# jd-opensource/xllm

Hardware: AMD Instinct MI355X
Metric: decode tokens/s, Qwen2-7B int8 bs=256 ctx=4096 (higher is better)
Workload: dtype int8; 1 GPU; qwen2_7b W8A8 int8 decode step, global_batch=256 ctx=4096, paged KV block=128 bf16, 28 layers + lm_head + argmax, random-init weights; global_batch=256, ctx=4096, per_gpu_batch=256, block_table=random placement of every sequence's pages in a pool of 1.1 x the pages in use, parallelism=tp1, layout=single, quant_fusion=True, micro_batches=1, hip_graph=True

## Files before the change

### xllm_amd/_lib.py

```python
from __future__ import annotations

import ctypes as C
import os

_HERE = os.path.dirname(os.path.abspath(__file__))
LIB_PATH = os.environ.get("XLLM_MI355_LIB") or os.path.join(_HERE, "lib", "libxllm_mi355.so")

vp, i64, i32, f32, sz = C.c_void_p, C.c_int64, C.c_int32, C.c_float, C.c_size_t
ci = C.c_int
u64 = C.c_uint64



class DecodeMetadata(C.Structure):
    _fields_ = ([(n, vp) for n in (
        "src_tokens", "src_positions", "src_new_cache_slots", "src_kv_seq_lens", "src_paged_kv_indptr",
        "src_paged_kv_indices", "src_paged_kv_last_page_len", "dst_tokens", "dst_positions", "dst_new_cache_slots",
        "dst_kv_seq_lens", "dst_kv_seq_lens_delta", "dst_paged_kv_indptr", "dst_paged_kv_indices",
        "dst_paged_kv_last_page_len")] +
        [(n, i64) for n in ("actual_num_tokens", "padded_num_tokens", "actual_batch_size", "actual_indices_size")] +
        [("dst_block_table", vp), ("dst_kv_lens", vp), ("max_blocks_per_seq", i64), ("padded_batch_size", i64)])



# ... 47 lines not shown
    "xllm_mi355_act_and_mul_dynamic_int8_quant": ([vp, vp, vp, i64, i64, ci, ci, vp], ci),
    "xllm_mi355_act_and_mul_dynamic_int8_quant_live": ([vp, vp, vp, i64, i64, ci, ci, vp, i64, vp], ci),
    "xllm_mi355_scaled_quantize": ([vp, vp, vp, i64, i64, ci, vp], ci),
    "xllm_mi355_scaled_matmul": ([vp, vp, vp, vp, vp, vp, vp, i64, i64, i64, ci, vp], ci),
    "xllm_mi355_scaled_matmul_add": ([vp, vp, vp, vp, vp, vp, vp, i64, i64, i64, ci, vp], ci),
    "xllm_mi355_add16": ([vp, vp, vp, i64, ci, vp], ci),
    "xllm_mi355_set_gemm_workspace": ([vp, sz], ci),
    "xllm_mi355_set_gemm_workspace_for_stream": ([vp, vp, sz], ci),
    "xllm_mi355_scaled_matmul_add_rms_norm": ([vp, vp, vp, vp, vp, vp, vp, f32, vp, vp, vp, i64, i64, i64, ci, vp], ci),
    "xllm_mi355_pack_weight_i8": ([vp, vp, i64, i64, vp], ci),
    "xllm_mi355_scaled_matmul_packed": ([vp, vp, vp, vp, vp, vp, vp, i64, i64, i64, ci, vp, sz, vp], ci),
    "xllm_mi355_scaled_matmul_add_rms_norm_packed": ([vp, vp, vp, vp, vp, vp, vp, f32, vp, vp, vp, i64, i64, i64, ci, vp, sz,
                                                      vp], ci),
    "xllm_mi355_scaled_matmul_gate_up_act": ([vp, vp, vp, vp, vp, vp, vp, vp, i64, i64, i64, ci, vp, sz, vp], ci),
    "xllm_mi355_quantize_with_row_amax": ([vp, vp, vp, vp, i64, i64, ci, vp], ci),
    "xllm_mi355_static_scaled_fp8_quant": ([vp, vp, vp, i64, ci, vp], ci),
    "xllm_mi355_fp8_scaled_quantize": ([vp, vp, vp, vp, i64, ci, vp], ci),
    "xllm_mi355_fp8_scaled_quantize_ws": ([vp, vp, vp, i64, ci, vp, sz, vp], ci),
    "xllm_mi355_fp8_scaled_matmul": ([vp, vp, vp, i64, vp, i64, vp, vp, i64, i64, i64, ci, vp], ci),
    "xllm_mi355_pack_weight_fp8": ([vp, vp, i64, i64, vp], ci),
    "xllm_mi355_fp8_scaled_matmul_packed": ([vp, vp, vp, i64, vp, i64, vp, vp, i64, i64, i64, ci, vp, sz, vp], ci),
    "xllm_mi355_matmul": ([vp, vp, vp, vp, i64, i64, i64, ci, vp], ci),
    "xllm_mi355_pack_weight_16": ([vp, vp, i64, i64, vp], ci),
    "xllm_mi355_matmul_packed": ([vp, vp, vp, vp, i64, i64, i64, ci, vp, sz, vp], ci),
    "xllm_mi355_matmul_gate_up_act": ([vp, vp, vp, vp, i64, i64, i64, ci, vp, sz, vp], ci),
    "xllm_mi355_matmul_argmax_workspace_bytes": ([i64, i64], sz),
    "xllm_mi355_matmul_argmax_packed": ([vp, vp, vp, vp, vp, i64, i64, i64, ci, vp, sz, vp], ci),
    "xllm_mi355_prefill_attention": ([vp, vp, vp, vp, vp, vp, i64, i64, i64, i64, i64, i64, i64, i64, f32, ci, i64,
                                      ci, vp], ci),
    "xllm_mi355_paged_decode_attention_int8": ([vp, vp, vp, vp, vp, vp, vp, vp, i64, i64, i64, i64, i64, i64, i64, i64,
# ... 76 lines not shown
```

### xllm_amd/csrc/gemm.hip

```cpp
#include <stdlib.h>

#include "gemm_types.h"

namespace xm {

constexpr int BM = 128, BN = 128, BKB = 128;

template <int KIND, bool SPLITK, int KB, int MINW>
__global__ __launch_bounds__(256, MINW) void gemm_kernel(const uint8_t* __restrict__ A_, const uint8_t* __restrict__ W_,
                                                      int M_, int N, int64_t Kb, int m_tiles, int n_tiles,
                                                      int ksteps_per_split, GemmEpi epi) {
  const uint8_t* A = A_;
  const uint8_t* W = W_;
  int M = M_;
  void* out_base = epi.out;
  using MT = MmaTraits<KIND>;
  using acc_t = typename MT::acc_t;
  constexpr int CPR = KB / 16;
  constexpr int NST = BM * CPR / 256;
  __shared__ __attribute__((aligned(16))) uint8_t lds[2][2][BM * KB];
  auto SW = [](int row) { return CPR == 8 ? ((row >> 1) & 7) : ((row >> 2) & 3); };

  const int tid = threadIdx.x, lane = tid & 63, wave = tid >> 6;
  const int wm = wave >> 1, wn = wave & 1;
// ... 771 lines not shown
  if (N % 256 != 0 || K % 128 != 0 || ((uintptr_t)a % 16) || ((uintptr_t)act_out % 16) || ((uintptr_t)w_scale % 16))
    return XM_ERR_UNSUPPORTED;
  if (M == 0) return XM_OK;
  GemmEpi epi{a_scale, M, w_scale, N, bias, nullptr, nullptr, dtype == XM_BF16, nullptr, 0};
  epi.gate_up = 1;
  epi.act_out = act_out;
  epi.row_amax = row_amax;
  if (w_packed && M <= 512) {
    const int rc = launch_gemm_ws_i8(a, w_packed, M, N, K, epi, workspace, ws_bytes, nullptr, (hipStream_t)stream);
    if (rc != XM_ERR_UNSUPPORTED) return rc;
  }
  if (!w || ((uintptr_t)w % 16)) return XM_ERR_UNSUPPORTED;
  return launch_gemm_p8<kI8>(a, w, M, N, K, epi, nullptr, 0, 1, (hipStream_t)stream);
}

int xllm_mi355_fp8_scaled_matmul(const uint8_t* a, const uint8_t* w, const float* a_scale, int64_t a_scale_numel,
                                 const float* w_scale, int64_t w_scale_numel, const void* bias, void* out, int64_t M,
                                 int64_t N, int64_t K, int out_dtype, void* stream) {
  if (!a || !w || !a_scale || !w_scale || !out || M < 0 || N < 0 || K <= 0) return XM_ERR_INVALID;
  if (out_dtype != XM_BF16 && out_dtype != XM_F16) return XM_ERR_UNSUPPORTED;
  if ((a_scale_numel != 1 && a_scale_numel != M) || (w_scale_numel != 1 && w_scale_numel != N)) return XM_ERR_INVALID;
  if (K % 128 != 0 || ((uintptr_t)a % 16) || ((uintptr_t)w % 16)) return XM_ERR_UNSUPPORTED;
  GemmEpi epi{a_scale, a_scale_numel, w_scale, w_scale_numel, bias, out, nullptr, out_dtype == XM_BF16, nullptr, 0};
  void* ws = nullptr;
  size_t ws_bytes = 0;
  gemm_ws_for(stream, &ws, &ws_bytes);
  return launch_gemm<kFP8>(a, w, M, N, K, epi, ws, ws_bytes, (hipStream_t)stream);
}

int xllm_mi355_pack_weight_fp8(const uint8_t* w, uint8_t* packed, int64_t N, int64_t K, void* stream) {
// ... 172 lines not shown
```

### xllm_amd/csrc/gemm_types.h

```cpp
#pragma once
#include <type_traits>

#include "common.h"

namespace xm {

typedef int i32x4_t __attribute__((ext_vector_type(4)));
typedef int i32x16_t __attribute__((ext_vector_type(16)));
typedef float f32x16_t __attribute__((ext_vector_type(16)));
typedef __bf16 gbf16x8_t __attribute__((ext_vector_type(8)));
typedef _Float16 gf16x8_t __attribute__((ext_vector_type(8)));

enum GemmKind { kI8 = 0, kFP8 = 1, kBF16 = 2, kF16 = 3 };

template <int KIND>
struct MmaTraits;
template <>
struct MmaTraits<kI8> {
  using acc_t = i32x16_t;
  static __device__ __forceinline__ acc_t zero() { return acc_t{0}; }
  static __device__ __forceinline__ acc_t mma(const uint4& a, const uint4& b, acc_t c) {
    i32x4_t av = {(int)a.x, (int)a.y, (int)a.z, (int)a.w}, bv = {(int)b.x, (int)b.y, (int)b.z, (int)b.w};
    return __builtin_amdgcn_mfma_i32_32x32x32_i8(av, bv, c, 0, 0, 0);
  }
// ... 47 lines not shown
  const int32_t* group_tiles;
  const int32_t* gather_rows;
  int gather_div;
  int gather_src_rows;
  int gate_up;
  void* act_out;
  float* row_amax;
  int w_policy;
  float* argmax_val;
  int32_t* argmax_idx;
  int argmax_slots;
  int slab_nt;
  int out_nt;
  const void* addend;
  int group_inline;
};

__device__ __forceinline__ bool argmax_better(float v, int i, float bv, int bi) {
  const bool vn = v != v, bn = bv != bv;
  if (vn || bn) return vn && (!bn || i < bi);
  return v > bv || (v == bv && i < bi);
}

struct GroupSlot { int e, off, cnt, tile; };
__device__ __forceinline__ bool group_locate(const GemmEpi& epi, int m_slots, int n_tiles, int bm, int lane, int& mt, int& nt,
                                             GroupSlot& gs) {
  const int b = blockIdx.x, xcd = b & 7, j = b >> 3;
  int used;
  int ct = 0, cr = 0, it = 0, ir = 0;
  int c4[4] = {0, 0, 0, 0};
// ... 149 lines not shown
               : "+v"(F[0]), "+v"(F[1]), "+v"(F[2]), "+v"(F[3]), "+v"(F[4]), "+v"(F[5]), "+v"(F[6]), "+v"(F[7]))

template <int KIND>
int launch_gemm_p8(const void* A, const void* W, int64_t M, int64_t N, int64_t Kb, GemmEpi epi, void* workspace,
                   size_t ws_bytes, int splits, hipStream_t s);

int launch_gemm_ws_i8(const void* A, const void* Wp, int64_t M, int64_t N, int64_t K, GemmEpi epi, void* workspace,
                      size_t ws_bytes, int* n_slabs, hipStream_t s);
int launch_gemm_ws_fp8(const void* A, const void* Wp, int64_t M, int64_t N, int64_t K, GemmEpi epi, void* workspace,
                       size_t ws_bytes, hipStream_t s);
int launch_gemm_ws_h16(const void* A, const void* Wp, int64_t M, int64_t N, int64_t Kb, GemmEpi epi, void* workspace,
                       size_t ws_bytes, hipStream_t s);
int launch_gemm_ws_h16_argmax(const void* A, const void* Wp, int64_t M, int64_t N, int64_t Kb, GemmEpi epi, int64_t* out_idx,
                              float* out_val, void* workspace, size_t ws_bytes, hipStream_t s);
int launch_pack_weight_i8(const void* W, void* Wp, int64_t N, int64_t K, hipStream_t s);

template <typename T>
int launch_gemm_wsb_dense(const void* x, const void* w, const void* bias, void* out, int64_t M, int64_t N, int64_t K,
                          void* workspace, size_t ws_bytes, hipStream_t s);
template <typename T>
int launch_gemm_wsb_grouped(const void* x, const void* w, const int32_t* counts, void* out, int64_t max_rows,
                            int64_t n_experts, int64_t N, int64_t K, const int32_t* row_index, int64_t index_div,
                            hipStream_t s);

}
```

### xllm_amd/csrc/gemm_ws.hip

```cpp
#include <stdlib.h>

#include "gemm_types.h"

namespace xm {

constexpr int WS_BK = 128;
constexpr int WS_FRAG = 1024;
#ifndef WS_W_AUX
#define WS_W_AUX 2
#endif

__global__ __launch_bounds__(256) void pack_weight_i8_kernel(const uint8_t* __restrict__ W, uint8_t* __restrict__ Wp,
                                                             int64_t N, int64_t K) {
  const int64_t chunks_per_row = K / 16, total = N * chunks_per_row;
  const int64_t KT = K / WS_BK;
  for (int64_t i = (int64_t)blockIdx.x * blockDim.x + threadIdx.x; i < total; i += (int64_t)gridDim.x * blockDim.x) {
    const int64_t n = i / chunks_per_row, c = i - n * chunks_per_row;
    const int64_t g = n >> 4, r = n & 15, kt = c >> 3, ks = (c >> 2) & 1, kq = c & 3;
    const uint4 v = *reinterpret_cast<const uint4*>(W + n * K + c * 16);
    *reinterpret_cast<uint4*>(Wp + ((g * KT + kt) * 2 + ks) * WS_FRAG + (kq * 16 + r) * 16) = v;
  }
}

#define WS_BUFLOAD(DST, VOFF, RSRC, SOFF, IMM)                                             \
// ... 15 lines not shown
  int so_a, so_w;
  ws_lds_ptr_t dump;
  int nvalid_w;
  int w_nt;
};
template <int NDA, int NDW, int WNT = -1>
__device__ __forceinline__ void ws_dma_piece(const WsDma& d, const int (&voff_a)[8], const int (&voff_w)[8], int j) {
  if (j < NDA) __builtin_amdgcn_raw_ptr_buffer_load_lds(d.rsrc_a, d.dst_a + j * WS_FRAG, 16, voff_a[j], d.so_a, 0, 0);
  else if (WNT == 1 || (WNT < 0 && d.w_nt))
    __builtin_amdgcn_raw_ptr_buffer_load_lds(d.rsrc_w, (j - NDA) < d.nvalid_w ? d.dst_w + (j - NDA) * WS_FRAG : d.dump, 16,
                                             voff_w[j - NDA], d.so_w, 0, WS_W_AUX);
  else
    __builtin_amdgcn_raw_ptr_buffer_load_lds(d.rsrc_w, (j - NDA) < d.nvalid_w ? d.dst_w + (j - NDA) * WS_FRAG : d.dump, 16,
                                             voff_w[j - NDA], d.so_w, 0, 0);
}
template <int NDA, int NDW, int NG>
__device__ __forceinline__ void ws_dma_slot(const WsDma& d, const int (&voff_a)[8], const int (&voff_w)[8], int slot) {
  constexpr int ND = NDA + NDW;
  const int lo = slot * ND / (2 * NG), hi = (slot + 1) * ND / (2 * NG);
#pragma unroll
  for (int j = lo; j < hi; ++j) ws_dma_piece<NDA, NDW>(d, voff_a, voff_w, j);
}

template <int NDA, int NDW, int LO, int HI, int WNT = -1>
__device__ __forceinline__ void ws_dma_range(const WsDma& d, const int (&voff_a)[8], const int (&voff_w)[8], int slot, int nslots) {
  const int lo = LO + slot * (HI - LO) / nslots, hi = LO + (slot + 1) * (HI - LO) / nslots;
#pragma unroll
  for (int j = lo; j < hi; ++j) ws_dma_piece<NDA, NDW, WNT>(d, voff_a, voff_w, j);
}

template <int MB, int NG, int NDA, int NDW, int NG_LEFT>
__device__ __forceinline__ void ws_kstep1(i32x4_t (&acc)[MB][NG], u32x4 (&fw)[NG], const u32x4 (&a1)[MB], const WsDma& d,
                                          const int (&voff_a)[8], const int (&voff_w)[8]) {
  if constexpr (NG_LEFT > 0) {
    constexpr int ng = NG - NG_LEFT;
    asm volatile("s_waitcnt lgkmcnt(%1)" : "+v"(fw[ng]) : "n"(NG_LEFT - 1));
#pragma unroll
    for (int mb = 0; mb < MB; ++mb) WS_MFMA(acc[mb][ng], fw[ng], a1[mb]);
    ws_dma_slot<NDA, NDW, NG>(d, voff_a, voff_w, NG + ng);
    ws_kstep1<MB, NG, NDA, NDW, NG_LEFT - 1>(acc, fw, a1, d, voff_a, voff_w);
  }
}
template <int MB, int NG, int NDA, int NDW>
__device__ __forceinline__ void ws_compute(i32x4_t (&acc)[MB][NG], unsigned rw, unsigned ra0, unsigned ra1, const WsDma& d,
                                           const int (&voff_a)[8], const int (&voff_w)[8]) {
  u32x4 a0[MB], a1[MB], fw[NG];
#pragma unroll
  for (int mb = 0; mb < MB; ++mb) WS_DSR(a0[mb], ra0, mb * 16 * WS_BK);
#pragma unroll
  for (int mb = 0; mb < MB; ++mb) WS_DSR(a1[mb], ra1, mb * 16 * WS_BK);
#pragma unroll
  for (int ng = 0; ng < NG; ++ng) WS_DSR(fw[ng], rw, ng * 2 * WS_FRAG);
#pragma unroll
  for (int ng = 0; ng < NG; ++ng) {
    if (ng == 0) {
      if constexpr (MB == 4)
        asm volatile("s_waitcnt lgkmcnt(%5)" : "+v"(a0[0]), "+v"(a0[1]), "+v"(a0[2]), "+v"(a0[3]), "+v"(fw[0]) : "n"(NG - 1));
      else
        asm volatile("s_waitcnt lgkmcnt(%3)" : "+v"(a0[0]), "+v"(a0[1]), "+v"(fw[0]) : "n"(NG - 1));
    } else {
      asm volatile("s_waitcnt lgkmcnt(%1)" : "+v"(fw[ng]) : "n"(NG - 1));
    }
#pragma unroll
    for (int mb = 0; mb < MB; ++mb) WS_MFMA(acc[mb][ng], fw[ng], a0[mb]);
    WS_DSR(fw[ng], rw, ng * 2 * WS_FRAG + WS_FRAG);
    ws_dma_slot<NDA, NDW, NG>(d, voff_a, voff_w, ng);
  }
  if constexpr (MB == 4) asm volatile("" : "+v"(a1[0]), "+v"(a1[1]), "+v"(a1[2]), "+v"(a1[3]));
  else asm volatile("" : "+v"(a1[0]), "+v"(a1[1]));
  ws_kstep1<MB, NG, NDA, NDW, NG>(acc, fw, a1, d, voff_a, voff_w);
  __builtin_amdgcn_sched_barrier(0);
}


typedef float f32x4_t __attribute__((ext_vector_type(4)));
__device__ __forceinline__ f32x4_t ws_mma_fp8(const u32x4 w0, const u32x4 w1, const u32x4 a0, const u32x4 a1, f32x4_t c) {
  const gi32x8_t wv = {(int)w0.x, (int)w0.y, (int)w0.z, (int)w0.w, (int)w1.x, (int)w1.y, (int)w1.z, (int)w1.w};
  const gi32x8_t av = {(int)a0.x, (int)a0.y, (int)a0.z, (int)a0.w, (int)a1.x, (int)a1.y, (int)a1.z, (int)a1.w};
  return __builtin_amdgcn_mfma_scale_f32_16x16x128_f8f6f4(wv, av, c, 0, 0, 0, 0, 0, 0);
}
template <int NDA, int NDW, int NSLOTS>
__device__ __forceinline__ void ws_dma_slot_n(const WsDma& d, const int (&voff_a)[8], const int (&voff_w)[8], int slot) {
  constexpr int ND = NDA + NDW;
  const int lo = slot * ND / NSLOTS, hi = (slot + 1) * ND / NSLOTS;
#pragma unroll
// ... 214 lines not shown
  if (!wide) return;
  asm volatile("s_waitcnt lgkmcnt(0)" ::: "memory");
#pragma unroll
  for (int i = 0; i < MB * NG / 2; ++i) {
    const int idx = i * 64 + lane, row = idx / CH, c = idx % CH;
    const uint4 v = *reinterpret_cast<const uint4*>(tb + row * PITCH + c * 16);
    const int m = m_base + row;
    if (m < M && gw + (c >> 1) < g_live)
      *reinterpret_cast<uint4*>(reinterpret_cast<uint16_t*>(epi.out) + (int64_t)m * N + (g0 + gw) * 16 + c * 8) = v;
  }
}

template <int KIND, int MB, int NG, int WM, int WN, int NWV>
__device__ __forceinline__ void ws_epilogue_gate_up(typename WsAcc<KIND>::type (&acc)[MB][NG], const GemmEpi& epi, int M, int N,
                                                    int m_tile0, int wm, int wn, int lane, int tid, int ga0, int ga_live,
                                                    int n_groups_act, uint8_t* lds) {
  constexpr int G = WN * NG, GH = G / 2, ROWS = WM * MB * 16, PITCH = G * 32 + 16;
  static_assert(G % 2 == 0 && ROWS * PITCH + ROWS * 4 <= 160 * 1024, "gate_up tile");
  const int g4 = lane >> 4, ml = lane & 15;
  const bool out_bf16 = epi.out_bf16 != 0, has_bias = epi.bias != nullptr;
  unsigned* const rowmax = reinterpret_cast<unsigned*>(lds + ROWS * PITCH);
  for (int r = tid; r < ROWS; r += NWV * 64) rowmax[r] = 0u;
  float asv[MB];
#pragma unroll
  for (int mb = 0; mb < MB; ++mb) {
    const int m = m_tile0 + wm * MB * 16 + mb * 16 + ml;
    asv[mb] = KIND == kI8 ? epi.a_scale[m < M ? m : M - 1] : 1.0f;
  }
#pragma unroll
  for (int ng = 0; ng < NG; ++ng) {
    const int q = wn * NG + ng, half = q / GH, j = q % GH;
// ... 52 lines not shown
        const f16_t o0 = (f16_t)r0, o1 = (f16_t)r1;
        uint16_t o0h, o1h;
        __builtin_memcpy(&o0h, &o0, 2); __builtin_memcpy(&o1h, &o1, 2);
        ow[w] = (uint32_t)o0h | ((uint32_t)o1h << 16);
      }
      amax = fmaxf(amax, fmaxf(fabsf(r0), fabsf(r1)));
    }
    *reinterpret_cast<uint4*>(reinterpret_cast<uint16_t*>(epi.act_out) + (int64_t)m * I + (int64_t)(ga0 + j) * 16 + hc * 8) =
        make_uint4(ow[0], ow[1], ow[2], ow[3]);
#ifndef WS_ABL_GU_NOLDSATOMIC
    if (epi.row_amax) atomicMax(&rowmax[row], __float_as_uint(amax));
#endif
  }
  if (!epi.row_amax) return;
  __syncthreads();
  for (int r = tid; r < ROWS; r += NWV * 64) {
    const int m = m_tile0 + r;
#ifndef WS_ABL_GU_NOATOMIC
    if (m < M && rowmax[r]) atomicMax(reinterpret_cast<unsigned*>(epi.row_amax) + m, rowmax[r]);
#endif
  }
}


template <int KIND, int NWV, int WM, int WN, int MB, int NG, int DW>
__global__ __launch_bounds__(NWV * 64, 1) void gemm_ws_kernel(const uint8_t* __restrict__ A, const uint8_t* __restrict__ Wp,
                                                             int M, int N, int64_t K, int m_tiles, int n_tiles,
                                                             int kt_per_slice, int n_slices, GemmEpi epi,
                                                             int32_t* __restrict__ slabs, int stagger) {
  static_assert(NWV == 4 || NWV == 8, "one or two waves per SIMD");
  static_assert(WM * WN == NWV, "waves per workgroup");
  static_assert(MB == 2 || MB == 4, "row blocks per wave");
  static_assert(KIND == kI8 || KIND == kFP8 || KIND == kBF16 || KIND == kF16, "operand kinds");
  using acc_t = typename WsAcc<KIND>::type;
  constexpr int G = WN * NG;
  constexpr int NS = DW + 1;
  constexpr int SLOT_W = G * 2 * WS_FRAG, SLOT_A = WM * MB * 2 * WS_FRAG, SLOT = SLOT_W + SLOT_A;
  constexpr int NDW = (2 * G + NWV - 1) / NWV;
  constexpr int NDA = (2 * WM * MB) / NWV;
  constexpr bool PAD = (2 * G) % NWV != 0;
// ... 4 lines not shown
  __shared__ __attribute__((aligned(1024))) uint8_t lds[NS * SLOT + (PAD ? WS_FRAG : 0)];

  const int tid = threadIdx.x, lane = tid & 63;
  const int wave = __builtin_amdgcn_readfirstlane(tid >> 6);
  const int wm = wave / WN, wn = wave % WN;
  int mt, nt, slice;
  {
    const int b = blockIdx.x, x = b & 7, y = b >> 3;
    mt = y % m_tiles;
    const int rest = (y / m_tiles) * 8 + x;
    if (rest >= n_tiles * n_slices) return;
    nt = rest % n_tiles;
    slice = rest / n_tiles;
  }
  const int KT = (int)(K / WS_BK);
  const int w_nt = epi.w_policy ? epi.w_policy == 1 : m_tiles == 1;
  const int kt0 = slice * kt_per_slice;
  int kt1 = kt0 + kt_per_slice;
  kt1 = kt1 > KT ? KT : kt1;
  const int nk = kt1 - kt0;
  const int phase = stagger ? (int)(((unsigned)blockIdx.x >> 3) % (unsigned)nk) : 0;
#define WS_ROT(X_) ((X_) + phase >= nk ? (X_) + phase - nk : (X_) + phase)
  const int n_groups = N >> 4;
  const bool gu = KIND != kFP8 && epi.gate_up != 0;
  const int n_groups_act = n_groups >> 1;
  const int ga0 = gu ? (int)((int64_t)nt * n_groups_act / n_tiles) : 0;
  const int ga_live = gu ? (int)((int64_t)(nt + 1) * n_groups_act / n_tiles) - ga0 : 0;
  const int g0 = gu ? 0 : (int)((int64_t)nt * n_groups / n_tiles);
  const int g_live = gu ? n_groups : (int)((int64_t)(nt + 1) * n_groups / n_tiles) - g0;
  const int m_tile0 = mt * (WM * MB * 16), m_base = m_tile0 + wm * (MB * 16);

// ... 75 lines not shown
    __builtin_amdgcn_s_barrier();
    __builtin_amdgcn_sched_barrier(0);
    const int tn = t + DW, tc = tn < nk ? tn : nk - 1, ktn = kt0 + WS_ROT(tc);
    WsDma d;
    d.rsrc_a = WS_ABL_RSRC_A;
    d.rsrc_w = WS_ABL_RSRC_W;
    d.dst_w = lds3 + (tn % NS) * SLOT + wave * NDW * WS_FRAG;
    d.dst_a = lds3 + (tn % NS) * SLOT + SLOT_W + wave * NDA * WS_FRAG;
    d.so_a = ktn * WS_BK;
    d.so_w = ktn * (2 * WS_FRAG);
    d.dump = lds_dump;
    d.nvalid_w = nvalid_w;
    d.w_nt = w_nt;
    const unsigned so = (t % NS) * SLOT;
#ifndef WS_ABL_NOCOMPUTE
    if constexpr (KIND == kI8) ws_compute<MB, NG, NDA, NDW>(acc, rd_w + so, rd_a0 + so, rd_a1 + so, d, voff_a, voff_w);
    else if constexpr (KIND == kFP8) ws_compute_fp8<MB, NG, NDA, NDW>(acc, rd_w + so, rd_a0 + so, rd_a1 + so, d, voff_a, voff_w);
    else ws_compute_h16<KIND, MB, NG, NDA, NDW>(acc, rd_w + so, rd_a0 + so, rd_a1 + so, d, voff_a, voff_w);
#else
    WS_ISSUE(tn)
#endif
  }
#undef WS_ISSUE
#undef WS_ROT
  asm volatile("s_waitcnt vmcnt(0)" ::: "memory");
  if constexpr (KIND == kI8) {
    if constexpr (MB == 4)
      asm volatile("s_nop 15\n\ts_nop 15" : "+a"(acc[0][NG - 1]), "+a"(acc[1][NG - 1]), "+a"(acc[2][NG - 1]), "+a"(acc[3][NG - 1]));
    else
      asm volatile("s_nop 15\n\ts_nop 15" : "+a"(acc[0][NG - 1]), "+a"(acc[1][NG - 1]));
  }

  __builtin_amdgcn_s_barrier();
  if constexpr (KIND != kFP8 && (WN * NG) % 2 == 0) {
    if (gu) {
      ws_epilogue_gate_up<KIND, MB, NG, WM, WN, NWV>(acc, epi, M, N, m_tile0, wm, wn, lane, tid, ga0, ga_live, n_groups_act, lds);
      return;
    }
  }
  ws_epilogue<KIND, MB, NG>(acc, epi, slabs, slice, n_slices, M, N, m_base, g0, g_live, wn, lane, lds, wave, nt * WN + wn);
}

#ifdef WS8_TIMING
__device__ long long ws8_dbg[64];
#endif
template <int KIND, int NG, int DW, int NRD, int WNT>
__global__ __launch_bounds__(512, 1) void gemm_ws8s_kernel(const uint8_t* __restrict__ A, const uint8_t* __restrict__ Wp,
                                                          int M, int N, int64_t K, int m_tiles, int n_tiles,
                                                          int kt_per_slice, int n_slices, GemmEpi epi,
                                                          int32_t* __restrict__ slabs) {
  constexpr int NWV = 8, WM = 4, WN = 2, MB = 4;
// ... 191 lines not shown
    __builtin_amdgcn_s_barrier();
    WS8_T(4)
  }
#ifdef WS8_TIMING
  const long long t_loop_end = __builtin_readcyclecounter();
#endif
#undef WS8_DESC
#undef WS8_T
#undef WS8_ISSUE
  if (!grp) __builtin_amdgcn_s_barrier();
  asm volatile("s_waitcnt vmcnt(0)" ::: "memory");
  if constexpr (KIND == kI8)
    asm volatile("s_nop 15\n\ts_nop 15" : "+a"(acc[0][NG - 1]), "+a"(acc[1][NG - 1]), "+a"(acc[2][NG - 1]), "+a"(acc[3][NG - 1]));
  __builtin_amdgcn_s_barrier();
  if constexpr (KIND != kFP8) {
    if (gu) ws_epilogue_gate_up<KIND, MB, NG, WM, WN, NWV>(acc, epi, M, N, m_tile0, wm, wn, lane, tid, ga0, ga_live, n_groups_act, lds);
  }
  if (!gu) ws_epilogue<KIND, MB, NG>(acc, epi, slabs, slice, n_slices, M, N, m_base, g0, g_live, wn, lane, lds, wave, nt * WN + wn);
#ifdef WS8_TIMING
  {
    asm volatile("s_waitcnt vmcnt(0)" ::: "memory");
    const long long t_end = __builtin_readcyclecounter(), r_end = __builtin_amdgcn_s_memrealtime();
    const int sel = blockIdx.x == 0 ? 0 : (blockIdx.x == gridDim.x / 2 ? 1 : -1);
    if (sel >= 0 && (wave & 3) == 0 && lane == 0) {
      long long* o = ws8_dbg + sel * 32 + grp * 16;
      for (int i = 0; i < 5; ++i) o[i] = tacc[i];
      o[5] = nk;
      o[6] = t_loop - t_entry;
      o[7] = t_loop_end - t_loop;
      o[8] = t_end - t_loop_end;
      o[9] = r_end - r_entry;
// ... 55 lines not shown
    }
    uint2 pk;
    if (epi.out_bf16) { pk.x = pack2x16<true>(v[0], v[1]); pk.y = pack2x16<true>(v[2], v[3]); }
    else { pk.x = pack2x16<false>(v[0], v[1]); pk.y = pack2x16<false>(v[2], v[3]); }
    *reinterpret_cast<uint2*>(reinterpret_cast<uint16_t*>(epi.out) + idx) = pk;
  }
}

struct WsPlan { int waves, wm, wn, mb, ng, slices; };

XM_TUNE_VAR(f_kstagger, "XLLM_MI355_KSTAGGER", 1);
XM_TUNE_VAR(f_ws8s, "XLLM_MI355_WS8_STAGGER", 1);
XM_TUNE_VAR(f_wpolicy, "XLLM_MI355_WS_WPOLICY", 0);
XM_TUNE_VAR(f_slab_nt, "XLLM_MI355_SLAB_NT", 1);
static thread_local int g_argmax_slots_used = 0;
template <int KIND, int NWV, int WM, int WN, int MB, int NG, int DW>
int ws_launch_cfg(const void* A, const void* Wp, int64_t M, int64_t N, int64_t K, int slices, GemmEpi epi,
                         int32_t* slabs, hipStream_t s) {
  constexpr int G = WN * NG;
  const int m_tiles = (int)((M + WM * MB * 16 - 1) / (WM * MB * 16));
  const bool gu = epi.gate_up != 0;
  epi.w_policy = f_wpolicy;
  epi.slab_nt = f_slab_nt;
  if (gu && (G % 2 != 0 || KIND == kFP8)) return -1;
  const int n_groups = gu ? (int)(N / 32) : (int)(N / 16);
  const int KT = (int)(K / WS_BK);
  if (gu || epi.argmax_val) slices = 1;
  int per = (KT + slices - 1) / slices;
  slices = (KT + per - 1) / per;
  constexpr int GCAP = G;
  int n_tiles = gu ? (n_groups + G / 2 - 1) / (G / 2) : (n_groups + GCAP - 1) / GCAP;
  const int fit = 256 / (m_tiles * slices);
  if (fit > n_tiles) n_tiles = fit < n_groups ? fit : n_groups;
  const int rest = n_tiles * slices;
  const unsigned grid = (unsigned)(((rest + 7) / 8) * 8 * m_tiles);
  if (epi.argmax_val) {
    if (n_tiles * WN > epi.argmax_slots) return -2;
    g_argmax_slots_used = n_tiles * WN;
  }
  if constexpr (NWV == 8) {
#ifdef XM_TUNING
    if (!f_ws8s) {
      hipLaunchKernelGGL((gemm_ws_kernel<KIND, NWV, WM, WN, MB, NG, DW>), dim3(grid), dim3(NWV * 64), 0, s, (const uint8_t*)A,
                         (const uint8_t*)Wp, (int)M, (int)N, K, m_tiles, n_tiles, per, slices, epi, slabs, f_kstagger);
      return slices;
    }
#endif
    constexpr int ND8 = (2 * WN * NG + 7) / 8 + 4;
    const bool w_nt = epi.w_policy ? epi.w_policy == 1 : m_tiles == 1;
    if (w_nt)
      hipLaunchKernelGGL((gemm_ws8s_kernel<KIND, NG, DW, ND8 / 2, 1>), dim3(grid), dim3(512), 0, s, (const uint8_t*)A,
                         (const uint8_t*)Wp, (int)M, (int)N, K, m_tiles, n_tiles, per, slices, epi, slabs);
    else
      hipLaunchKernelGGL((gemm_ws8s_kernel<KIND, NG, DW, ND8 / 2, 0>), dim3(grid), dim3(512), 0, s, (const uint8_t*)A,
                         (const uint8_t*)Wp, (int)M, (int)N, K, m_tiles, n_tiles, per, slices, epi, slabs);
  } else {
    hipLaunchKernelGGL((gemm_ws_kernel<KIND, NWV, WM, WN, MB, NG, DW>), dim3(grid), dim3(NWV * 64), 0, s, (const uint8_t*)A,
                       (const uint8_t*)Wp, (int)M, (int)N, K, m_tiles, n_tiles, per, slices, epi, slabs, f_kstagger);
  }
  return slices;
}

static thread_local int f_ng = 0, f_sl = 0, f_rows = 0;
#ifdef XM_TUNING
struct WsShapePlan { int64_t N, K; int ng, slices; };
static WsShapePlan shape_plans[8];
static int n_shape_plans = 0;
#endif
static WsPlan ws_plan(int64_t M, int64_t N, int64_t K, bool can_slice, size_t ws_bytes, bool gu = false) {
  WsPlan p;
  p.waves = 4;
  if (M <= 32) { p.wm = 1; p.wn = 4; p.mb = 2; }
// ... 216 lines not shown
```

### xllm_amd/csrc/rowwise.hip

```cpp
#include "common.h"

namespace xm {

constexpr int kRowThreads = 256;
constexpr int kMaxVec = 4;

template <typename V>
__global__ __launch_bounds__(256) void reshape_paged_cache_kernel(
    const int32_t* __restrict__ slot_ids, const V* __restrict__ k, const V* __restrict__ v,
    V* __restrict__ kc, V* __restrict__ vc, int64_t row_v ,
    int64_t k_stride_v, int64_t v_stride_v, int64_t block_size, int64_t n_blocks) {
  const int64_t t = blockIdx.x;
  const int64_t slot = slot_ids[t];
  if (slot < 0) return;
  if (slot / block_size >= n_blocks) return;
  const V* ks = k + t * k_stride_v;
  V* kd = kc + slot * row_v;
  if (v) {
    const V* vs = v + t * v_stride_v;
    V* vd = vc + slot * row_v;
    for (int64_t i = threadIdx.x; i < row_v; i += blockDim.x) {
      kd[i] = ks[i];
      vd[i] = vs[i];
    }
// ... 1543 lines not shown
          wq |= ((uint32_t)(int)qv & 0xffu) << (8 * e);
        }
        pk[h] = wq;
      }
      u32x2* const dst = reinterpret_cast<u32x2*>(out_q + t * (int64_t)d + (int64_t)c * 8);
      const u32x2 qv2 = {pk[0], pk[1]};
      if (nt) __builtin_nontemporal_store(qv2, dst);
      else *dst = qv2;
    }
  }
  __syncthreads();
  if (threadIdx.x == 0) { out_s[t] = amax / 127.0f; row_amax[t] = 0.0f; }
}

template <typename T>
__global__ __launch_bounds__(256) void add16_kernel(T* __restrict__ out, const T* a, const T* b, int64_t n) {
  const int64_t nvec = n / 8;
  for (int64_t c = (int64_t)blockIdx.x * 256 + threadIdx.x; c < nvec; c += (int64_t)gridDim.x * 256) {
    RowVec<T> x, y, r;
    x.raw = reinterpret_cast<const uint4*>(a)[c];
    y.raw = reinterpret_cast<const uint4*>(b)[c];
#pragma unroll
    for (int j = 0; j < 8; ++j) r.set(j, x.get(j) + y.get(j));
    reinterpret_cast<uint4*>(out)[c] = r.raw;
  }
  if (blockIdx.x == 0)
    for (int64_t i = nvec * 8 + threadIdx.x; i < n; i += 256) out[i] = from_f32<T>(to_f32(a[i]) + to_f32(b[i]));
}

extern "C" {
// ... 133 lines not shown
```

### xllm_amd/ops.py

```python
from __future__ import annotations

from typing import Optional, Tuple

import ctypes as C
import os

import torch

from . import _lib
from ._lib import Mi355Error, check

_DT = {torch.float32: 0, torch.bfloat16: 1, torch.float16: 2}
_ACT = {"silu": 0, "gelu": 1, "gelu_tanh": 2}
FP8 = torch.float8_e4m3fn


def _stream() -> int:
    return torch.cuda.current_stream().cuda_stream


def _p(t: Optional[torch.Tensor]) -> int:
    return 0 if t is None else t.data_ptr()


# ... 354 lines not shown
            _row_amax_retired.append(amax)
        amax = torch.zeros(max(M, 16384), dtype=torch.float32, device=device)
        _row_amax[key] = amax
    return amax


_GATE_UP_FUSION = os.environ.get("XLLM_MI355_GATE_UP_FUSION", "1") == "1"


def scaled_matmul_silu_mul_quant(a, b, a_scale, b_scale, output_dtype=torch.bfloat16, bias=None, b_packed=None):
    _need_cuda(a, b, a_scale, b_scale)
    M, K = a.shape
    N = b.size(0)
    if not _GATE_UP_FUSION or N % 256 or K % 128 or not a.is_contiguous() or not b.is_contiguous() or M == 0:
        return None
    amax = _row_amax_scratch(a.device, M)
    I = N // 2
    act = torch.empty(M, I, dtype=output_dtype, device=a.device)
    rc = _lib.lib().xllm_mi355_scaled_matmul_gate_up_act(_p(a), _p(b), _p(b_packed), _p(a_scale.reshape(-1)),
                                                        _p(b_scale.reshape(-1)), _p(bias), _p(act), _p(amax), M, N, K,
                                                        _DT[output_dtype], 0, 0, _stream())
    if rc == -2:
        return None
    check(rc, "scaled_matmul_gate_up_act")
    q = torch.empty(M, I, dtype=torch.int8, device=a.device)
    qs = torch.empty(M, dtype=torch.float32, device=a.device)
    check(_lib.lib().xllm_mi355_quantize_with_row_amax(_p(act), _p(amax), _p(q), _p(qs), M, I, _DT[output_dtype], _stream()),
          "quantize_with_row_amax")
    return q, qs


def scaled_matmul_add_rms_norm(a, b, a_scale, b_scale, residual, norm_weight, eps: float, bias=None,
                               quantize: bool = True, b_packed=None):
# ... 619 lines not shown
```

Measured before the change: 19250 tokens/s.

## Replace atomic row-amax with per-tile partial maxima in gate-up quant path

Adds a packed gate_up GEMM entry point whose epilogue writes each N-tile's per-row activation max into a partials buffer instead of using atomics on a shared row_amax scratch. A new quantize kernel reduces the partials per row and quantizes the activation in the same launch, so the scratch no longer needs to be cleared after use. The weight non-temporal policy also becomes a template parameter of the workspace GEMM kernel, giving two instantiations and a compile-time flag in place of a runtime value. This trades atomic contention for an extra read of N/32 partials per row and a larger partials allocation on every call.

```diff
diff --git a/xllm_amd/_lib.py b/xllm_amd/_lib.py
--- a/xllm_amd/_lib.py
+++ b/xllm_amd/_lib.py
@@ -85,6 +85,7 @@
                                                       vp], ci),
     "xllm_mi355_scaled_matmul_gate_up_act": ([vp, vp, vp, vp, vp, vp, vp, vp, i64, i64, i64, ci, vp, sz, vp], ci),
     "xllm_mi355_quantize_with_row_amax": ([vp, vp, vp, vp, i64, i64, ci, vp], ci),
+    "xllm_mi355_scaled_matmul_gate_up_quant_packed": ([vp, vp, vp, vp, vp, vp, vp, i64, vp, vp, i64, i64, i64, ci, vp], ci),
     "xllm_mi355_static_scaled_fp8_quant": ([vp, vp, vp, i64, ci, vp], ci),
     "xllm_mi355_fp8_scaled_quantize": ([vp, vp, vp, vp, i64, ci, vp], ci),
     "xllm_mi355_fp8_scaled_quantize_ws": ([vp, vp, vp, i64, ci, vp, sz, vp], ci),
diff --git a/xllm_amd/csrc/gemm.hip b/xllm_amd/csrc/gemm.hip
--- a/xllm_amd/csrc/gemm.hip
+++ b/xllm_amd/csrc/gemm.hip
@@ -809,6 +809,29 @@
   return launch_gemm_p8<kI8>(a, w, M, N, K, epi, nullptr, 0, 1, (hipStream_t)stream);
 }
 
+int xllm_mi355_scaled_matmul_gate_up_quant_packed(const int8_t* a, const int8_t* w_packed, const float* a_scale,
+                                                  const float* w_scale, const void* bias, void* act, float* amax_parts,
+                                                  int64_t parts_cap, int8_t* out_q, float* out_scale, int64_t M, int64_t N,
+                                                  int64_t K, int dtype, void* stream) {
+  if (!a || !w_packed || !a_scale || !w_scale || !act || !amax_parts || !out_q || !out_scale || M < 0 || N <= 0 || K <= 0 ||
+      parts_cap <= 0)
+    return XM_ERR_INVALID;
+  if (dtype != XM_BF16 && dtype != XM_F16) return XM_ERR_UNSUPPORTED;
+  if (M > 512 || N % 256 != 0 || K % 128 != 0 || ((uintptr_t)a % 16) || ((uintptr_t)w_packed % 16) || ((uintptr_t)act % 16) ||
+      ((uintptr_t)w_scale % 16) || ((uintptr_t)out_q % 8))
+    return XM_ERR_UNSUPPORTED;
+  if (M == 0) return XM_OK;
+  GemmEpi epi{a_scale, M, w_scale, N, bias, nullptr, nullptr, dtype == XM_BF16, nullptr, 0};
+  epi.gate_up = 1;
+  epi.act_out = act;
+  epi.row_amax = amax_parts;
+  epi.row_amax_parts = parts_cap > (1 << 30) ? (1 << 30) : (int)parts_cap;
+  const int rc = launch_gemm_ws_i8(a, w_packed, M, N, K, epi, nullptr, 0, nullptr, (hipStream_t)stream);
+  if (rc != XM_OK) return rc;
+  return launch_quantize_with_row_amax_parts(act, amax_parts, ws_last_amax_parts(), out_q, out_scale, M, N / 2, dtype,
+                                             (hipStream_t)stream);
+}
+
 int xllm_mi355_fp8_scaled_matmul(const uint8_t* a, const uint8_t* w, const float* a_scale, int64_t a_scale_numel,
                                  const float* w_scale, int64_t w_scale_numel, const void* bias, void* out, int64_t M,
                                  int64_t N, int64_t K, int out_dtype, void* stream) {
diff --git a/xllm_amd/csrc/gemm_types.h b/xllm_amd/csrc/gemm_types.h
--- a/xllm_amd/csrc/gemm_types.h
+++ b/xllm_amd/csrc/gemm_types.h
@@ -85,6 +85,7 @@
   int out_nt;
   const void* addend;
   int group_inline;
+  int row_amax_parts;
 };
 
 __device__ __forceinline__ bool argmax_better(float v, int i, float bv, int bi) {
@@ -264,6 +265,9 @@
 int launch_gemm_ws_h16_argmax(const void* A, const void* Wp, int64_t M, int64_t N, int64_t Kb, GemmEpi epi, int64_t* out_idx,
                               float* out_val, void* workspace, size_t ws_bytes, hipStream_t s);
 int launch_pack_weight_i8(const void* W, void* Wp, int64_t N, int64_t K, hipStream_t s);
+int ws_last_amax_parts();
+int launch_quantize_with_row_amax_parts(const void* act, const float* parts, int n_parts, int8_t* out_q, float* out_scale,
+                                        int64_t n_tokens, int64_t d, int dtype, hipStream_t s);
 
 template <typename T>
 int launch_gemm_wsb_dense(const void* x, const void* w, const void* bias, void* out, int64_t M, int64_t N, int64_t K,
@@ -274,3 +278,9 @@
                             hipStream_t s);
 
 }
+
+extern "C" XM_API int xllm_mi355_scaled_matmul_gate_up_quant_packed(const int8_t* a, const int8_t* w_packed, const float* a_scale,
+                                                                    const float* w_scale, const void* bias, void* act,
+                                                                    float* amax_parts, int64_t parts_cap, int8_t* out_q,
+                                                                    float* out_scale, int64_t M, int64_t N, int64_t K, int dtype,
+                                                                    void* stream);
diff --git a/xllm_amd/csrc/gemm_ws.hip b/xllm_amd/csrc/gemm_ws.hip
--- a/xllm_amd/csrc/gemm_ws.hip
+++ b/xllm_amd/csrc/gemm_ws.hip
@@ -53,12 +53,12 @@
     __builtin_amdgcn_raw_ptr_buffer_load_lds(d.rsrc_w, (j - NDA) < d.nvalid_w ? d.dst_w + (j - NDA) * WS_FRAG : d.dump, 16,
                                              voff_w[j - NDA], d.so_w, 0, 0);
 }
-template <int NDA, int NDW, int NG>
+template <int NDA, int NDW, int NG, int WNT = -1>
 __device__ __forceinline__ void ws_dma_slot(const WsDma& d, const int (&voff_a)[8], const int (&voff_w)[8], int slot) {
   constexpr int ND = NDA + NDW;
   const int lo = slot * ND / (2 * NG), hi = (slot + 1) * ND / (2 * NG);
 #pragma unroll
-  for (int j = lo; j < hi; ++j) ws_dma_piece<NDA, NDW>(d, voff_a, voff_w, j);
+  for (int j = lo; j < hi; ++j) ws_dma_piece<NDA, NDW, WNT>(d, voff_a, voff_w, j);
 }
 
 template <int NDA, int NDW, int LO, int HI, int WNT = -1>
@@ -68,7 +68,7 @@
   for (int j = lo; j < hi; ++j) ws_dma_piece<NDA, NDW, WNT>(d, voff_a, voff_w, j);
 }
 
-template <int MB, int NG, int NDA, int NDW, int NG_LEFT>
+template <int MB, int NG, int NDA, int NDW, int WNT, int NG_LEFT>
 __device__ __forceinline__ void ws_kstep1(i32x4_t (&acc)[MB][NG], u32x4 (&fw)[NG], const u32x4 (&a1)[MB], const WsDma& d,
                                           const int (&voff_a)[8], const int (&voff_w)[8]) {
   if constexpr (NG_LEFT > 0) {
@@ -76,11 +76,11 @@
     asm volatile("s_waitcnt lgkmcnt(%1)" : "+v"(fw[ng]) : "n"(NG_LEFT - 1));
 #pragma unroll
     for (int mb = 0; mb < MB; ++mb) WS_MFMA(acc[mb][ng], fw[ng], a1[mb]);
-    ws_dma_slot<NDA, NDW, NG>(d, voff_a, voff_w, NG + ng);
-    ws_kstep1<MB, NG, NDA, NDW, NG_LEFT - 1>(acc, fw, a1, d, voff_a, voff_w);
-  }
-}
-template <int MB, int NG, int NDA, int NDW>
+    ws_dma_slot<NDA, NDW, NG, WNT>(d, voff_a, voff_w, NG + ng);
+    ws_kstep1<MB, NG, NDA, NDW, WNT, NG_LEFT - 1>(acc, fw, a1, d, voff_a, voff_w);
+  }
+}
+template <int MB, int NG, int NDA, int NDW, int WNT = -1>
 __device__ __forceinline__ void ws_compute(i32x4_t (&acc)[MB][NG], unsigned rw, unsigned ra0, unsigned ra1, const WsDma& d,
                                            const int (&voff_a)[8], const int (&voff_w)[8]) {
   u32x4 a0[MB], a1[MB], fw[NG];
@@ -103,11 +103,11 @@
 #pragma unroll
     for (int mb = 0; mb < MB; ++mb) WS_MFMA(acc[mb][ng], fw[ng], a0[mb]);
     WS_DSR(fw[ng], rw, ng * 2 * WS_FRAG + WS_FRAG);
-    ws_dma_slot<NDA, NDW, NG>(d, voff_a, voff_w, ng);
+    ws_dma_slot<NDA, NDW, NG, WNT>(d, voff_a, voff_w, ng);
   }
   if constexpr (MB == 4) asm volatile("" : "+v"(a1[0]), "+v"(a1[1]), "+v"(a1[2]), "+v"(a1[3]));
   else asm volatile("" : "+v"(a1[0]), "+v"(a1[1]));
-  ws_kstep1<MB, NG, NDA, NDW, NG>(acc, fw, a1, d, voff_a, voff_w);
+  ws_kstep1<MB, NG, NDA, NDW, WNT, NG>(acc, fw, a1, d, voff_a, voff_w);
   __builtin_amdgcn_sched_barrier(0);
 }
 
@@ -352,7 +352,7 @@
 template <int KIND, int MB, int NG, int WM, int WN, int NWV>
 __device__ __forceinline__ void ws_epilogue_gate_up(typename WsAcc<KIND>::type (&acc)[MB][NG], const GemmEpi& epi, int M, int N,
                                                     int m_tile0, int wm, int wn, int lane, int tid, int ga0, int ga_live,
-                                                    int n_groups_act, uint8_t* lds) {
+                                                    int n_groups_act, uint8_t* lds, int nt) {
   constexpr int G = WN * NG, GH = G / 2, ROWS = WM * MB * 16, PITCH = G * 32 + 16;
   static_assert(G % 2 == 0 && ROWS * PITCH + ROWS * 4 <= 160 * 1024, "gate_up tile");
   const int g4 = lane >> 4, ml = lane & 15;
@@ -435,6 +435,12 @@
   }
   if (!epi.row_amax) return;
   __syncthreads();
+  if (epi.row_amax_parts) {
+    unsigned* const part = reinterpret_cast<unsigned*>(epi.row_amax) + (int64_t)nt * M;
+    for (int r = tid; r < ROWS; r += NWV * 64)
+      if (m_tile0 + r < M) part[m_tile0 + r] = rowmax[r];
+    return;
+  }
   for (int r = tid; r < ROWS; r += NWV * 64) {
     const int m = m_tile0 + r;
 #ifndef WS_ABL_GU_NOATOMIC
@@ -444,7 +450,7 @@
 }
 
 
-template <int KIND, int NWV, int WM, int WN, int MB, int NG, int DW>
+template <int KIND, int NWV, int WM, int WN, int MB, int NG, int DW, int WNT>
 __global__ __launch_bounds__(NWV * 64, 1) void gemm_ws_kernel(const uint8_t* __restrict__ A, const uint8_t* __restrict__ Wp,
                                                              int M, int N, int64_t K, int m_tiles, int n_tiles,
                                                              int kt_per_slice, int n_slices, GemmEpi epi,
@@ -479,7 +485,7 @@
     slice = rest / n_tiles;
   }
   const int KT = (int)(K / WS_BK);
-  const int w_nt = epi.w_policy ? epi.w_policy == 1 : m_tiles == 1;
+  constexpr int w_nt = WNT;
   const int kt0 = slice * kt_per_slice;
   int kt1 = kt0 + kt_per_slice;
   kt1 = kt1 > KT ? KT : kt1;
@@ -585,7 +591,7 @@
     d.w_nt = w_nt;
     const unsigned so = (t % NS) * SLOT;
 #ifndef WS_ABL_NOCOMPUTE
-    if constexpr (KIND == kI8) ws_compute<MB, NG, NDA, NDW>(acc, rd_w + so, rd_a0 + so, rd_a1 + so, d, voff_a, voff_w);
+    if constexpr (KIND == kI8) ws_compute<MB, NG, NDA, NDW, WNT>(acc, rd_w + so, rd_a0 + so, rd_a1 + so, d, voff_a, voff_w);
     else if constexpr (KIND == kFP8) ws_compute_fp8<MB, NG, NDA, NDW>(acc, rd_w + so, rd_a0 + so, rd_a1 + so, d, voff_a, voff_w);
     else ws_compute_h16<KIND, MB, NG, NDA, NDW>(acc, rd_w + so, rd_a0 + so, rd_a1 + so, d, voff_a, voff_w);
 #else
@@ -605,7 +611,7 @@
   __builtin_amdgcn_s_barrier();
   if constexpr (KIND != kFP8 && (WN * NG) % 2 == 0) {
     if (gu) {
-      ws_epilogue_gate_up<KIND, MB, NG, WM, WN, NWV>(acc, epi, M, N, m_tile0, wm, wn, lane, tid, ga0, ga_live, n_groups_act, lds);
+      ws_epilogue_gate_up<KIND, MB, NG, WM, WN, NWV>(acc, epi, M, N, m_tile0, wm, wn, lane, tid, ga0, ga_live, n_groups_act, lds, nt);
       return;
     }
   }
@@ -827,7 +833,7 @@
     asm volatile("s_nop 15\n\ts_nop 15" : "+a"(acc[0][NG - 1]), "+a"(acc[1][NG - 1]), "+a"(acc[2][NG - 1]), "+a"(acc[3][NG - 1]));
   __builtin_amdgcn_s_barrier();
   if constexpr (KIND != kFP8) {
-    if (gu) ws_epilogue_gate_up<KIND, MB, NG, WM, WN, NWV>(acc, epi, M, N, m_tile0, wm, wn, lane, tid, ga0, ga_live, n_groups_act, lds);
+    if (gu) ws_epilogue_gate_up<KIND, MB, NG, WM, WN, NWV>(acc, epi, M, N, m_tile0, wm, wn, lane, tid, ga0, ga_live, n_groups_act, lds, nt);
   }
   if (!gu) ws_epilogue<KIND, MB, NG>(acc, epi, slabs, slice, n_slices, M, N, m_base, g0, g_live, wn, lane, lds, wave, nt * WN + wn);
 #ifdef WS8_TIMING
@@ -913,6 +919,8 @@
 XM_TUNE_VAR(f_wpolicy, "XLLM_MI355_WS_WPOLICY", 0);
 XM_TUNE_VAR(f_slab_nt, "XLLM_MI355_SLAB_NT", 1);
 static thread_local int g_argmax_slots_used = 0;
+static thread_local int g_amax_parts_used = 0;
+int ws_last_amax_parts() { return g_amax_parts_used; }
 template <int KIND, int NWV, int WM, int WN, int MB, int NG, int DW>
 int ws_launch_cfg(const void* A, const void* Wp, int64_t M, int64_t N, int64_t K, int slices, GemmEpi epi,
                          int32_t* slabs, hipStream_t s) {
@@ -937,24 +945,35 @@
     if (n_tiles * WN > epi.argmax_slots) return -2;
     g_argmax_slots_used = n_tiles * WN;
   }
+  if (gu && epi.row_amax_parts) {
+    if (n_tiles > epi.row_amax_parts) return -2;
+    g_amax_parts_used = n_tiles;
+  }
+  const bool w_nt = epi.w_policy ? epi.w_policy == 1 : m_tiles == 1;
   if constexpr (NWV == 8) {
 #ifdef XM_TUNING
     if (!f_ws8s) {
-      hipLaunchKernelGGL((gemm_ws_kernel<KIND, NWV, WM, WN, MB, NG, DW>), dim3(grid), dim3(NWV * 64), 0, s, (const uint8_t*)A,
-                         (const uint8_t*)Wp, (int)M, (int)N, K, m_tiles, n_tiles, per, slices, epi, slabs, f_kstagger);
+      if (w_nt)
+        hipLaunchKernelGGL((gemm_ws_kernel<KIND, NWV, WM, WN, MB, NG, DW, 1>), dim3(grid), dim3(NWV * 64), 0, s, (const uint8_t*)A,
+                           (const uint8_t*)Wp, (int)M, (int)N, K, m_tiles, n_tiles, per, slices, epi, slabs, f_kstagger);
+      else
+        hipLaunchKernelGGL((gemm_ws_kernel<KIND, NWV, WM, WN, MB, NG, DW, 0>), dim3(grid), dim3(NWV * 64), 0, s, (const uint8_t*)A,
+                           (const uint8_t*)Wp, (int)M, (int)N, K, m_tiles, n_tiles, per, slices, epi, slabs, f_kstagger);
       return slices;
     }
 #endif
     constexpr int ND8 = (2 * WN * NG + 7) / 8 + 4;
-    const bool w_nt = epi.w_policy ? epi.w_policy == 1 : m_tiles == 1;
     if (w_nt)
       hipLaunchKernelGGL((gemm_ws8s_kernel<KIND, NG, DW, ND8 / 2, 1>), dim3(grid), dim3(512), 0, s, (const uint8_t*)A,
                          (const uint8_t*)Wp, (int)M, (int)N, K, m_tiles, n_tiles, per, slices, epi, slabs);
     else
       hipLaunchKernelGGL((gemm_ws8s_kernel<KIND, NG, DW, ND8 / 2, 0>), dim3(grid), dim3(512), 0, s, (const uint8_t*)A,
                          (const uint8_t*)Wp, (int)M, (int)N, K, m_tiles, n_tiles, per, slices, epi, slabs);
+  } else if (w_nt) {
+    hipLaunchKernelGGL((gemm_ws_kernel<KIND, NWV, WM, WN, MB, NG, DW, 1>), dim3(grid), dim3(NWV * 64), 0, s, (const uint8_t*)A,
+                       (const uint8_t*)Wp, (int)M, (int)N, K, m_tiles, n_tiles, per, slices, epi, slabs, f_kstagger);
   } else {
-    hipLaunchKernelGGL((gemm_ws_kernel<KIND, NWV, WM, WN, MB, NG, DW>), dim3(grid), dim3(NWV * 64), 0, s, (const uint8_t*)A,
+    hipLaunchKernelGGL((gemm_ws_kernel<KIND, NWV, WM, WN, MB, NG, DW, 0>), dim3(grid), dim3(NWV * 64), 0, s, (const uint8_t*)A,
                        (const uint8_t*)Wp, (int)M, (int)N, K, m_tiles, n_tiles, per, slices, epi, slabs, f_kstagger);
   }
   return slices;
diff --git a/xllm_amd/csrc/rowwise.hip b/xllm_amd/csrc/rowwise.hip
--- a/xllm_amd/csrc/rowwise.hip
+++ b/xllm_amd/csrc/rowwise.hip
@@ -1581,6 +1581,82 @@
 }
 
 template <typename T>
+__global__ __launch_bounds__(512) void quantize_with_row_amax_parts_kernel(const T* __restrict__ act,
+                                                                          const unsigned* __restrict__ parts, int n_parts,
+                                                                          int8_t* __restrict__ out_q, float* __restrict__ out_s,
+                                                                          int d, int nt) {
+  typedef unsigned u32x4 __attribute__((ext_vector_type(4)));
+  typedef unsigned u32x2 __attribute__((ext_vector_type(2)));
+  __shared__ unsigned wmax[8];
+  const int64_t t = blockIdx.x, M = gridDim.x;
+  const int tid = threadIdx.x;
+  const int nvec = d / 8;
+  const u32x4* x = reinterpret_cast<const u32x4*>(act + t * (int64_t)d);
+  constexpr int U = 6;
+  u32x4 vv[U];
+#pragma unroll
+  for (int u = 0; u < U; ++u) {
+    const int c = tid + u * 512;
+    if (c < nvec) vv[u] = nt ? __builtin_nontemporal_load(&x[c]) : x[c];
+  }
+  unsigned b = 0u;
+  for (int p = tid; p < n_parts; p += 512) b = max(b, parts[(int64_t)p * M + t]);
+#pragma unroll
+  for (int o = 32; o >= 1; o >>= 1) b = max(b, (unsigned)__shfl_xor((int)b, o));
+  if ((tid & 63) == 0) wmax[tid >> 6] = b;
+  __syncthreads();
+#pragma unroll
+  for (int w = 0; w < 8; ++w) b = max(b, wmax[w]);
+  const float amax = __uint_as_float(b);
+  const float qinv = (amax > 1e-10f) ? 127.0f / amax : 0.0f;
+  for (int c0 = tid; c0 < nvec; c0 += U * 512) {
+    if (c0 != tid) {
+#pragma unroll
+      for (int u = 0; u < U; ++u) {
+        const int c = c0 + u * 512;
+        if (c < nvec) vv[u] = nt ? __builtin_nontemporal_load(&x[c]) : x[c];
+      }
+    }
+#pragma unroll
+    for (int u = 0; u < U; ++u) {
+      const int c = c0 + u * 512;
+      if (c >= nvec) break;
+      const u32x4 v = vv[u];
+      uint32_t pk[2];
+#pragma unroll
+      for (int h = 0; h < 2; ++h) {
+        uint32_t wq = 0;
+#pragma unroll
+        for (int e = 0; e < 4; ++e) {
+          const uint32_t word = v[h * 2 + (e >> 1)];
+          const float r = half_bits_to_f32<T>((e & 1) ? (word >> 16) : (word & 0xffffu));
+          const float qv = fmaxf(-127.0f, fminf(127.0f, rintf(r * qinv)));
+          wq |= ((uint32_t)(int)qv & 0xffu) << (8 * e);
+        }
+        pk[h] = wq;
+      }
+      u32x2* const dst = reinterpret_cast<u32x2*>(out_q + t * (int64_t)d + (int64_t)c * 8);
+      const u32x2 qv2 = {pk[0], pk[1]};
+      if (nt) __builtin_nontemporal_store(qv2, dst);
+      else *dst = qv2;
+    }
+  }
+  if (tid == 0) out_s[t] = amax / 127.0f;
+}
+
+namespace xm {
+int launch_quantize_with_row_amax_parts(const void* act, const float* parts, int n_parts, int8_t* out_q, float* out_scale,
+                                        int64_t n_tokens, int64_t d, int dtype, hipStream_t s) {
+  if (n_tokens == 0) return XM_OK;
+  XM_DISPATCH_HALF(dtype, T,
+                   hipLaunchKernelGGL((quantize_with_row_amax_parts_kernel<T>), dim3((unsigned)n_tokens), dim3(512), 0, s,
+                                      (const T*)act, reinterpret_cast<const unsigned*>(parts), n_parts, out_q, out_scale, (int)d,
+                                      (n_tokens * d * 2 > (48ll << 20)) ? 1 : 0));
+  return hip_check_launch();
+}
+}
+
+template <typename T>
 __global__ __launch_bounds__(256) void add16_kernel(T* __restrict__ out, const T* a, const T* b, int64_t n) {
   const int64_t nvec = n / 8;
   for (int64_t c = (int64_t)blockIdx.x * 256 + threadIdx.x; c < nvec; c += (int64_t)gridDim.x * 256) {
diff --git a/xllm_amd/ops.py b/xllm_amd/ops.py
--- a/xllm_amd/ops.py
+++ b/xllm_amd/ops.py
@@ -392,9 +392,19 @@
     N = b.size(0)
     if not _GATE_UP_FUSION or N % 256 or K % 128 or not a.is_contiguous() or not b.is_contiguous() or M == 0:
         return None
-    amax = _row_amax_scratch(a.device, M)
     I = N // 2
     act = torch.empty(M, I, dtype=output_dtype, device=a.device)
+    if b_packed is not None and M <= 512:
+        parts = torch.empty(N // 32, M, dtype=torch.float32, device=a.device)
+        q = torch.empty(M, I, dtype=torch.int8, device=a.device)
+        qs = torch.empty(M, dtype=torch.float32, device=a.device)
+        rc = _lib.lib().xllm_mi355_scaled_matmul_gate_up_quant_packed(
+            _p(a), _p(b_packed), _p(a_scale.reshape(-1)), _p(b_scale.reshape(-1)), _p(bias), _p(act), _p(parts), N // 32,
+            _p(q), _p(qs), M, N, K, _DT[output_dtype], _stream())
+        if rc != -2:
+            check(rc, "scaled_matmul_gate_up_quant_packed")
+            return q, qs
+    amax = _row_amax_scratch(a.device, M)
     rc = _lib.lib().xllm_mi355_scaled_matmul_gate_up_act(_p(a), _p(b), _p(b_packed), _p(a_scale.reshape(-1)),
                                                         _p(b_scale.reshape(-1)), _p(bias), _p(act), _p(amax), M, N, K,
                                                         _DT[output_dtype], 0, 0, _stream())
```

Result: faster. 19470 tokens/s, median of 6 (+1.1%).
